# Bardli/RMem_ocu

Measured on AMD Instinct MI355X. Metric: frames/sec (whole node) 480p VOS, N=8 memory bank, higher is better.
Workload: dtype bf16; 1 GPU; davis17_480p_r50_N8; clip_frames=80, job_clips=64, clip_feeder=static, objects=3, memory_bank=1+7, gap=5, clips_in_flight_per_gpu=24, clips_per_group=8, step_unit=batch, parallelism=clip-parallel x1, weights=synthetic (no checkpoint offline), hipgraphs=True, frames_from=HBM, encoder_lookahead=2

## Files before the change

### rmem_ocu_amd/csrc/bottleneck.hip

```cpp
#include "common.h"
#include "lds_dma.h"
#include "../../include/rmem.h"
#include <stdlib.h>

namespace {

constexpr int BM = 64, N1 = 256, BK = 64;
constexpr int R1_BYTES = N1 * BK * 2, CP = 132, R2_BYTES = 16 * CP * 4, R3_BYTES = 32768;
static_assert(R2_BYTES >= BM * BK * 2, "the A panel shares the staging region");
constexpr int LDS_BYTES = R1_BYTES + R2_BYTES + R3_BYTES;

struct BnParams {
  const e16* b; const e16* x2; const e16* w3; const float* b3; const e16* res; e16* y;
  const e16* w1; const float* b1; e16* a2;
  int M, K1, KT, N2;
  int Ho, Wo, HoWo, H2, W2, Cin2, stride2;
  long b_bytes, x2_bytes;
};

template <int N2, bool DUAL>
__global__ __launch_bounds__(256) void k_bneck_chain(BnParams p) {
  constexpr int NB2 = N2 / 32;
  constexpr int NST = N2 == 64 ? 4 : 2;
  constexpr int TN2 = N2 / 32;
  constexpr int NRES = DUAL ? 0 : 8;
  static_assert(NST * N2 * BK * 2 <= R3_BYTES, "W1' ring");
  __shared__ __attribute__((aligned(16))) char smem[LDS_BYTES];
  char* const R1 = smem;
  char* const R2 = smem + R1_BYTES;
  char* const R3 = smem + R1_BYTES + R2_BYTES;

  const int tid = threadIdx.x, lane = tid & 63;
  const int wave = __builtin_amdgcn_readfirstlane(tid >> 6);
  const int wm = wave >> 1, wn = wave & 1;
  const int fr = lane & 15, fc = lane >> 4;
  const int m0 = blockIdx.x * BM;

  int a_off[2], a_off2[2], w3_off[8], w1_off[NB2];
#pragma unroll
  for (int i = 0; i < 2; ++i) {
    const int r = 16 * wave + 8 * i + (lane >> 3);
    const int c = (lane & 7) ^ ((r >> 1) & 7);
    const int m = m0 + r;
    a_off[i] = m < p.M ? (m * p.K1 + c * 8) * 2 : OOB;
    a_off2[i] = OOB;
    if (DUAL && m < p.M) {
      const int img = m / p.HoWo, rem = m - img * p.HoWo;
      const int ho = rem / p.Wo, wo = rem - ho * p.Wo;
      a_off2[i] = (((img * p.H2 + ho * p.stride2) * p.W2 + wo * p.stride2) * p.Cin2 + c * 8) * 2;
    }
  }
#pragma unroll
  for (int i = 0; i < 8; ++i) {
    const int r = 64 * wave + 8 * i + (lane >> 3);
    const int c = (lane & 7) ^ ((r >> 1) & 7);
    w3_off[i] = (r * p.KT + c * 8) * 2;
  }
#pragma unroll
  for (int i = 0; i < NB2; ++i) {
    const int r = (N2 / 4) * wave + 8 * i + (lane >> 3);
    const int c = (lane & 7) ^ ((r >> 1) & 7);
    w1_off[i] = (r * N1 + c * 8) * 2;
  }
  const rsrc_t rs_b = make_rsrc(p.b, p.b_bytes), rs_x2 = make_rsrc(DUAL ? p.x2 : p.b, DUAL ? p.x2_bytes : 0);
  const rsrc_t rs_w3 = make_rsrc(p.w3, (long)N1 * p.KT * 2), rs_w1 = make_rsrc(p.w1, (long)N2 * N1 * 2);
  const int nk1 = p.K1 / BK, nk = p.KT / BK;

  auto issue1 = [&](int kt) {
    if (DUAL && kt >= nk1) {
#pragma unroll
      for (int i = 0; i < 2; ++i) buf_load_lds16(rs_x2, (lptr_t)(R2 + (16 * wave + 8 * i) * 128), a_off2[i], (kt - nk1) * (BK * 2));
    } else {
#pragma unroll
      for (int i = 0; i < 2; ++i) buf_load_lds16(rs_b, (lptr_t)(R2 + (16 * wave + 8 * i) * 128), a_off[i], kt * (BK * 2));
    }
#pragma unroll
    for (int i = 0; i < 8; ++i) buf_load_lds16(rs_w3, (lptr_t)(R1 + (64 * wave + 8 * i) * 128), w3_off[i], kt * (BK * 2));
  };
  auto issue2 = [&](int kt, int stage) {
#pragma unroll
    for (int i = 0; i < NB2; ++i)
      buf_load_lds16(rs_w1, (lptr_t)(R3 + stage * (N2 * BK * 2) + ((N2 / 4) * wave + 8 * i) * 128), w1_off[i], kt * (BK * 2));
  };

  issue1(0);
#pragma unroll
  for (int s = 0; s < NST; ++s) issue2(s, s);
  __builtin_amdgcn_sched_barrier(0);
  e16x8 resv[NRES > 0 ? NRES : 1];
  const int erow = tid >> 4, ecv = tid & 15;
  if constexpr (!DUAL) {
#pragma unroll
    for (int q = 0; q < 8; ++q) {
      const int m = min(m0 + (q >> 1) * 16 + erow, p.M - 1);
      resv[q] = *reinterpret_cast<const e16x8*>(p.res + (long)m * N1 + (q & 1) * 128 + ecv * 8);
    }
  }
  f32x4 bias3[2][2], bias1[2];
#pragma unroll
  for (int h = 0; h < 2; ++h) {
    bias3[h][0] = *reinterpret_cast<const f32x4*>(p.b3 + h * 128 + ecv * 8);
    bias3[h][1] = *reinterpret_cast<const f32x4*>(p.b3 + h * 128 + ecv * 8 + 4);
  }
  constexpr int VPR2 = N2 / 8;
  bias1[0] = *reinterpret_cast<const f32x4*>(p.b1 + (tid % VPR2) * 8);
  bias1[1] = *reinterpret_cast<const f32x4*>(p.b1 + (tid % VPR2) * 8 + 4);
  __builtin_amdgcn_sched_barrier(0);

  f32x4 acc[2][8];
#pragma unroll
  for (int i = 0; i < 2; ++i)
#pragma unroll
    for (int j = 0; j < 8; ++j) acc[i][j] = f32x4{0.f, 0.f, 0.f, 0.f};

  for (int kt = 0; kt < nk; ++kt) {
    if (kt == 0) {
      asm volatile("s_waitcnt vmcnt(%0)" ::"n"(NST * NB2 + NRES + 6) : "memory");
    } else {
      __builtin_amdgcn_s_barrier();
      issue1(kt);
      asm volatile("s_waitcnt vmcnt(0)" ::: "memory");
    }
    __builtin_amdgcn_s_barrier();
    const e16* As = reinterpret_cast<const e16*>(R2);
    const e16* Bs = reinterpret_cast<const e16*>(R1);
#pragma unroll
    for (int ks = 0; ks < 2; ++ks) {
      e16x8 af[2], bfr[8];
#pragma unroll
      for (int i = 0; i < 2; ++i) af[i] = *reinterpret_cast<const e16x8*>(&As[swz(wm * 32 + i * 16 + fr, 4 * ks + fc)]);
#pragma unroll
      for (int j = 0; j < 8; ++j) bfr[j] = *reinterpret_cast<const e16x8*>(&Bs[swz(wn * 128 + j * 16 + fr, 4 * ks + fc)]);
#pragma unroll
      for (int i = 0; i < 2; ++i)
#pragma unroll
        for (int j = 0; j < 8; ++j) acc[i][j] = RMEM_MFMA_16x16x32(af[i], bfr[j], acc[i][j], 0, 0, 0);
    }
  }
  __syncthreads();

  float* Cs = reinterpret_cast<float*>(R2);
  e16* Yt = reinterpret_cast<e16*>(R1);
#pragma unroll
  for (int q = 0; q < 8; ++q) {
    const int g = q >> 1, h = q & 1;
    if (wm == (g >> 1) && wn == h) {
#pragma unroll
      for (int j = 0; j < 8; ++j)
#pragma unroll
        for (int r = 0; r < 4; ++r) Cs[(fc * 4 + r) * CP + j * 16 + fr] = acc[g & 1][j][r];
    }
    __syncthreads();
    {
      const int rt = g * 16 + erow, m = m0 + rt, n = h * 128 + ecv * 8;
      const float* c = Cs + erow * CP + ecv * 8;
      const f32x4 c0 = *reinterpret_cast<const f32x4*>(c), c1 = *reinterpret_cast<const f32x4*>(c + 4);
      const f32x4 b0 = bias3[h][0], b1 = bias3[h][1];
      float v[8] = {c0[0] + b0[0], c0[1] + b0[1], c0[2] + b0[2], c0[3] + b0[3], c1[0] + b1[0], c1[1] + b1[1], c1[2] + b1[2], c1[3] + b1[3]};
      e16x8 o;
#pragma unroll
      for (int j = 0; j < 8; ++j) {
        if constexpr (!DUAL) v[j] += (float)resv[q][j];
        o[j] = (e16)fmaxf(v[j], 0.f);
      }
      if (m < p.M) *reinterpret_cast<e16x8*>(p.y + (long)m * N1 + n) = o;
      *reinterpret_cast<e16x8*>(&Yt[(n >> 6) * (BM * BK) + swz(rt, (n >> 3) & 7)]) = o;
    }
    __syncthreads();
  }

  f32x4 acc2[2][TN2];
#pragma unroll
  for (int i = 0; i < 2; ++i)
#pragma unroll
    for (int j = 0; j < TN2; ++j) acc2[i][j] = f32x4{0.f, 0.f, 0.f, 0.f};
  if constexpr (DUAL) asm volatile("s_waitcnt vmcnt(0)" ::: "memory");
  if constexpr (DUAL) __syncthreads();
#pragma unroll
  for (int kt = 0; kt < 4; ++kt) {
    const int stage = kt % NST;
    if (kt >= NST) {
      if (kt + 1 < 4) asm volatile("s_waitcnt vmcnt(%0)" ::"n"(NB2) : "memory");
      else asm volatile("s_waitcnt vmcnt(0)" ::: "memory");
      __builtin_amdgcn_s_barrier();
    }
    const e16* As = Yt + kt * (BM * BK);
    const e16* Bs = reinterpret_cast<const e16*>(R3 + stage * (N2 * BK * 2));
#pragma unroll
    for (int ks = 0; ks < 2; ++ks) {
      e16x8 af[2], bfr[TN2];
#pragma unroll
      for (int i = 0; i < 2; ++i) af[i] = *reinterpret_cast<const e16x8*>(&As[swz(wm * 32 + i * 16 + fr, 4 * ks + fc)]);
#pragma unroll
      for (int j = 0; j < TN2; ++j) bfr[j] = *reinterpret_cast<const e16x8*>(&Bs[swz(wn * (N2 / 2) + j * 16 + fr, 4 * ks + fc)]);
#pragma unroll
      for (int i = 0; i < 2; ++i)
#pragma unroll
        for (int j = 0; j < TN2; ++j) acc2[i][j] = RMEM_MFMA_16x16x32(af[i], bfr[j], acc2[i][j], 0, 0, 0);
    }
    if (kt + NST < 4) {
      __syncthreads();
      issue2(kt + NST, stage);
    }
  }
  __syncthreads();

  constexpr int CP2 = N2 + 4;
  static_assert(16 * CP2 * 4 <= R2_BYTES, "second staging buffer");
#pragma unroll
  for (int g = 0; g < 4; ++g) {
    if (wm == (g >> 1)) {
#pragma unroll
      for (int j = 0; j < TN2; ++j)
#pragma unroll
        for (int r = 0; r < 4; ++r) Cs[(fc * 4 + r) * CP2 + wn * (N2 / 2) + j * 16 + fr] = acc2[g & 1][j][r];
    }
    __syncthreads();
    if (tid < 16 * VPR2) {
      const int row = tid / VPR2, cv = tid % VPR2;
      const int m = m0 + g * 16 + row, n = cv * 8;
      const float* c = Cs + row * CP2 + n;
      const f32x4 c0 = *reinterpret_cast<const f32x4*>(c), c1 = *reinterpret_cast<const f32x4*>(c + 4);
      const f32x4 b0 = bias1[0], b1 = bias1[1];
      const float v[8] = {c0[0] + b0[0], c0[1] + b0[1], c0[2] + b0[2], c0[3] + b0[3], c1[0] + b1[0], c1[1] + b1[1], c1[2] + b1[2], c1[3] + b1[3]};
      e16x8 o;
#pragma unroll
      for (int j = 0; j < 8; ++j) o[j] = (e16)fmaxf(v[j], 0.f);
      if (m < p.M) *reinterpret_cast<e16x8*>(p.a2 + (long)m * N2 + n) = o;
    }
    __syncthreads();
  }
}

bool al16(const void* q) { return ((uintptr_t)q % 16) == 0; }

}

extern "C" int RMEM_API(rmem_bneck_chain)(const rmem_bneck_chain_desc* d, const void* b, const void* x2, const void* w3, const float* bias3,
                                          const void* res, void* y, const void* w1, const float* bias1, void* a2, void* stream) {
  RMEM_REQUIRE(d && b && w3 && bias3 && y && w1 && bias1 && a2, "rmem_bneck_chain: null argument");
  RMEM_REQUIRE(d->batch >= 1 && d->Ho > 0 && d->Wo > 0 && d->K1 > 0 && d->K1 % 64 == 0 && d->Cout == 256 && (d->N2 == 64 || d->N2 == 128),
               "rmem_bneck_chain: K1 must be a multiple of 64, Cout 256, N2 64 or 128");
  RMEM_REQUIRE((x2 != nullptr) != (res != nullptr), "rmem_bneck_chain: exactly one of res (identity shortcut) and x2 (1x1 shortcut) must be given");
  RMEM_REQUIRE(!x2 || (d->Cin2 > 0 && d->Cin2 % 64 == 0 && d->stride2 >= 1 && d->H2 >= (d->Ho - 1) * d->stride2 + 1 && d->W2 >= (d->Wo - 1) * d->stride2 + 1),
               "rmem_bneck_chain: the 1x1 shortcut needs Cin2 % 64 == 0 and an H2 x W2 map that covers the strided samples");
  RMEM_REQUIRE(al16(b) && al16(x2) && al16(w3) && al16(bias3) && al16(res) && al16(y) && al16(w1) && al16(bias1) && al16(a2),
               "rmem_bneck_chain: operands must be 16-byte aligned");
  BnParams p;
  p.b = (const e16*)b; p.x2 = (const e16*)x2; p.w3 = (const e16*)w3; p.b3 = bias3; p.res = (const e16*)res; p.y = (e16*)y;
  p.w1 = (const e16*)w1; p.b1 = bias1; p.a2 = (e16*)a2;
  p.Ho = d->Ho; p.Wo = d->Wo; p.HoWo = d->Ho * d->Wo;
  const long M = (long)d->batch * p.HoWo;
  p.K1 = d->K1; p.KT = d->K1 + (x2 ? d->Cin2 : 0); p.N2 = d->N2;
  p.H2 = d->H2; p.W2 = d->W2; p.Cin2 = d->Cin2; p.stride2 = d->stride2;
  p.b_bytes = M * d->K1 * 2;
  p.x2_bytes = x2 ? (long)d->batch * d->H2 * d->W2 * d->Cin2 * 2 : 0;
  const long lim = (1L << 31) - (1L << 22);
  RMEM_REQUIRE(M < (1L << 30) && p.b_bytes < lim && p.x2_bytes < lim, "rmem_bneck_chain: an operand exceeds the 2 GB a buffer descriptor addresses");
  p.M = (int)M;
  const dim3 grid((unsigned)((M + BM - 1) / BM));
  hipStream_t s = (hipStream_t)stream;
  if (x2) {
    if (d->N2 == 64) hipLaunchKernelGGL((k_bneck_chain<64, true>), grid, dim3(256), 0, s, p);
    else hipLaunchKernelGGL((k_bneck_chain<128, true>), grid, dim3(256), 0, s, p);
  } else {
    if (d->N2 == 64) hipLaunchKernelGGL((k_bneck_chain<64, false>), grid, dim3(256), 0, s, p);
    else hipLaunchKernelGGL((k_bneck_chain<128, false>), grid, dim3(256), 0, s, p);
  }
  return rmem_check_launch("rmem_bneck_chain");
}
```

### rmem_ocu_amd/encoder_batch.py

```python
from __future__ import annotations

import os
from typing import Dict, Tuple

import torch

from . import ops
from .pack import R50_BLOCKS, R50_STRIDES
from .runtime import BF16, F32, _out


class _PtrInput:

    def _init_ptrs(self, B: int, device):
        self.img_ptrs = torch.tensor([self.img_in[i].data_ptr() for i in range(B)], dtype=torch.int64).to(device)
        self._ptr_ring = ops.PinnedRing(4, (B,), torch.int64, device)
        self._ptrs_set = False

    def _input_op(self):
        return ops.image_ptrs_to_nhwc8(self.img_ptrs, self.img8, H=self.H, W=self.W, images=self.B)

    def set_frames(self, frames, stream: int):
        assert len(frames) == self.B
        host = self._ptr_ring.next()
        for i, f in enumerate(frames):
            assert f.dtype == F32 and f.is_contiguous() and f.numel() == 3 * self.H * self.W
            host[i] = f.data_ptr()
        self._ptr_ring.upload(self.img_ptrs, self.B * 8, stream)
        self._ptrs_set = True

    def point_at_img_in(self, stream: int):
        if self._ptrs_set:
            self.set_frames([self.img_in[i] for i in range(self.B)], stream)
            self._ptrs_set = False


class BatchEncoder(_PtrInput):
    def __init__(self, P: Dict[str, torch.Tensor], in_hw: Tuple[int, int], batch: int, device):
        if 'pe.w' in P:
            raise ops.RmemError('BatchEncoder covers the ResNet-50 encoder')
        self.P, self.B, self.dev = P, batch, device
        H, W = in_hw
        self.H, self.W = H, W
        B = batch
        self.H2, self.W2 = _out(H, 7, 2, 3), _out(W, 7, 2, 3)
        self.H4, self.W4 = _out(self.H2, 3, 2, 1), _out(self.W2, 3, 2, 1)
        self.H8, self.W8 = _out(self.H4, 3, 2, 1), _out(self.W4, 3, 2, 1)
        self.H16, self.W16 = _out(self.H8, 3, 2, 1), _out(self.W8, 3, 2, 1)
        M4, M8, L = self.H4 * self.W4, self.H8 * self.W8, self.H16 * self.W16
        dt16 = P['stem.w'].dtype
        e = lambda *shape, dt=None: torch.empty(*shape, dtype=dt or dt16, device=device)
        self.img_in = e(B, 3, H, W, dt=F32)
        self._init_ptrs(B, device)
        self.stem4 = os.environ.get('RMEM_STEM', 'pool') != 'rowrun' and 'stem.w4' in P
        if self.stem4:
            hp, wp = ops.stem_padded_size(H, W)
            self.img4 = torch.zeros(B, hp, wp, 4, dtype=dt16, device=device)
        else:
            self.img8 = e(B, H * W, 8)
        self.stem_pool = self.stem4 and os.environ.get('RMEM_STEM', 'pool') == 'pool'
        self.stem = None if self.stem_pool else e(B, self.H2 * self.W2, 64)
        self.pool = e(B, M4, 64)
        self.x4 = [e(B, M4, 256), e(B, M4, 256)]
        self.x8 = [e(B, M8, 512), e(B, M8, 512)]
        self.x16 = [e(B, L, 1024), e(B, L, 1024)]
        self.mid_a = e(B * M4 * 128)
        self.mid_b = e(B * M4 * 64)
        self.conv_ws = torch.empty(16 * B * L * 256, dtype=F32, device=device)
        self._prog = None
        self.enc_out = (self.x4[(R50_BLOCKS[0] - 1) % 2], self.x8[(R50_BLOCKS[1] - 1) % 2], self.x16[(R50_BLOCKS[2] - 1) % 2])

    def _conv(self, *a, **kw):
        return ops.conv2d(*a, ws=self.conv_ws, batch=self.B, **kw)

    def prog(self) -> list:
        if self._prog is not None:
            return self._prog
        P, B, o = self.P, self.B, []
        nsplit = int(os.environ.get('RMEM_ENC_FRONT_SPLIT', '1'))
        if nsplit < 1 or B % nsplit:
            nsplit = 1
        chain_on = os.environ.get('RMEM_NO_BNECK_CHAIN', '0') != '1'
        block_on = chain_on and os.environ.get('RMEM_NO_BNECK_BLOCK', '0') != '1'
        direct3 = () if os.environ.get('RMEM_NO_DIRECT_CONV3', '0') == '1' else ((64, 128) if os.environ.get('RMEM_DIRECT_CONV3_128') == '1' else (64,))
        blocks = [(li, bi) for li, nblk in enumerate(R50_BLOCKS, start=1) for bi in range(nblk)]
        outs = [self.x4, self.x8, self.x16]
        M4 = self.H4 * self.W4
        if nsplit > 1 and getattr(self, 'mid_a128', None) is None:
            self.mid_a128 = torch.empty(B * M4 * 128, dtype=self.pool.dtype, device=self.dev)

        def sub(t, per_image, b0, nb):
            return t.reshape(-1)[b0 * per_image:(b0 + nb) * per_image]

        def stem(b0, nb):
            q = []
            conv = lambda *a_, **kw: ops.conv2d(*a_, ws=self.conv_ws, batch=nb, **kw)
            pool = sub(self.pool, M4 * 64, b0, nb)
            if self.stem4:
                hp, wp = ops.stem_padded_size(self.H, self.W)
                img4 = sub(self.img4, hp * wp * 4, b0, nb)
                q.append(ops.image_ptrs_to_nhwc4p(self.img_ptrs[b0:], img4, H=self.H, W=self.W, images=nb))
                if self.stem_pool:
                    q.append(ops.stem7x7s2_pool(img4, P['stem.w4'], P['stem.b'], pool, H=self.H, W=self.W, images=nb))
                else:
                    st = sub(self.stem, self.H2 * self.W2 * 64, b0, nb)
                    q.append(ops.stem7x7s2(img4, P['stem.w4'], P['stem.b'], st, H=self.H, W=self.W, images=nb))
                    q.append(ops.maxpool3x3s2(st, pool, H=self.H2, W=self.W2, C=64, images=nb))
            else:
                img8 = sub(self.img8, self.H * self.W * 8, b0, nb)
                st = sub(self.stem, self.H2 * self.W2 * 64, b0, nb)
                q.append(ops.image_ptrs_to_nhwc8(self.img_ptrs[b0:], img8, H=self.H, W=self.W, images=nb))
                q.append(conv(img8, P['stem.w'], P['stem.b'], st, H=self.H, W=self.W, Cin=8, Cout=64, KH=7, KW=7, stride=2, pad=3, relu=True))
                q.append(ops.maxpool3x3s2(st, pool, H=self.H2, W=self.W2, C=64, images=nb))
            return q

        def run_blocks(idxs, b0, nb, x, hw, cin, conv1_done):
            q = []
            conv = lambda *a_, **kw: ops.conv2d(*a_, ws=self.conv_ws, batch=nb, **kw)
            h, w = hw
            for idx in idxs:
                li, bi = blocks[idx]
                stride = R50_STRIDES[li - 1]
                planes = 64 * 2 ** (li - 1)
                p = f'encoder.layer{li}.{bi}'
                s = stride if bi == 0 else 1
                ho, wo = _out(h, 3, s, 1), _out(w, 3, s, 1)
                xs = sub(x, h * w * cin, b0, nb)
                y = sub(outs[li - 1][bi % 2], ho * wo * planes * 4, b0, nb)
                abuf = self.mid_a128 if (nsplit > 1 and li == 2 and bi == 0) else self.mid_a
                a = sub(abuf, h * w * planes, b0, nb)
                bb = sub(self.mid_b, ho * wo * planes, b0, nb)
                dual = (p + '.c3ds.w') in P
                nxt = blocks[idx + 1] if idx + 1 < len(blocks) else None
                if block_on and li == 1 and s == 1 and not conv1_done and cin == (64 if dual else 256):
                    kw = {}
                    if nxt == (2, 0):
                        pn = 'encoder.layer2.0'
                        nbuf = self.mid_a128 if nsplit > 1 else self.mid_a
                        kw = dict(w1n=P[pn + '.conv1.w'], bias1n=P[pn + '.conv1.b'], a_next=sub(nbuf, ho * wo * 128, b0, nb))
                        conv1_done = True
                    q.append(ops.bneck_block64(xs, P[p + '.conv1.w'], P[p + '.conv1.b'], P[p + '.conv2.w'], P[p + '.conv2.b'],
                                               P[p + ('.c3ds.w' if dual else '.conv3.w')], P[p + ('.c3ds.b' if dual else '.conv3.b')], y,
                                               H=h, W=w, Cin=cin, images=nb, **kw))
                    x, (h, w), cin = outs[li - 1][bi % 2], (ho, wo), planes * 4
                    continue
                if not conv1_done:
                    q.append(conv(xs, P[p + '.conv1.w'], P[p + '.conv1.b'], a, H=h, W=w, Cin=cin, Cout=planes, relu=True))
                conv1_done = False
                if planes in direct3 and s == 1:
                    q.append(ops.conv3x3_direct(a, P[p + '.conv2.w'], P[p + '.conv2.b'], bb, H=h, W=w, C=planes, images=nb, relu=True))
                else:
                    q.append(conv(a, P[p + '.conv2.w'], P[p + '.conv2.b'], bb, H=h, W=w, Cin=planes, Cout=planes, KH=3, KW=3, stride=s, pad=1,
                                  relu=True))
                if chain_on and li == 1 and nxt is not None:
                    pn = f'encoder.layer{nxt[0]}.{nxt[1]}'
                    n2 = 64 * 2 ** (nxt[0] - 1)
                    nbuf = self.mid_a128 if (nsplit > 1 and nxt == (2, 0)) else self.mid_a
                    a_next = sub(nbuf, ho * wo * n2, b0, nb)
                    kw = dict(x2=xs, H2=h, W2=w, Cin2=cin, stride2=s) if dual else dict(residual=xs)
                    q.append(ops.bneck_chain(bb, P[p + ('.c3ds.w' if dual else '.conv3.w')], P[p + ('.c3ds.b' if dual else '.conv3.b')], y,
                                             P[pn + '.conv1.w'], P[pn + '.conv1.b'], a_next, H=ho, W=wo, K1=planes, N2=n2, batch=nb, **kw))
                    conv1_done = True
                elif dual:
                    q.append(ops.conv1x1_dual(bb, xs, P[p + '.c3ds.w'], P[p + '.c3ds.b'], y, H=ho, W=wo, Cin=planes, Cout=planes * 4,
                                              H2=h, W2=w, Cin2=cin, stride2=s, relu=True, batch=nb))
                else:
                    q.append(conv(bb, P[p + '.conv3.w'], P[p + '.conv3.b'], y, H=ho, W=wo, Cin=planes, Cout=planes * 4, residual=xs, relu=True))
                x, (h, w), cin = outs[li - 1][bi % 2], (ho, wo), planes * 4
            return q, x, (h, w), cin, conv1_done

        n1 = R50_BLOCKS[0]
        nb = B // nsplit
        for k in range(nsplit):
            o += stem(k * nb, nb)
            q, x, hw, cin, c1 = run_blocks(range(n1), k * nb, nb, self.pool, (self.H4, self.W4), 64, False)
            o += q
        q, x, hw, cin, c1 = run_blocks(range(n1, len(blocks)), 0, B, x, hw, cin, c1)
        o += q
        self._prog = o
        return o


class SwinBatchEncoder(_PtrInput):

    def __init__(self, P: Dict[str, torch.Tensor], in_hw: Tuple[int, int], batch: int, device):
        if 'pe.w' not in P:
            raise ops.RmemError('SwinBatchEncoder covers the Swin-B encoder')
        self.P, self.B, self.dev = P, batch, device
        H, W = in_hw
        if H % 4 or W % 4:
            raise ops.RmemError('Swin-B path: network size must be a multiple of 4')
        self.H, self.W = H, W
        B = batch
        self.H4, self.W4 = H // 4, W // 4
        self.H8, self.W8 = (self.H4 + 1) // 2, (self.W4 + 1) // 2
        self.H16, self.W16 = (self.H8 + 1) // 2, (self.W8 + 1) // 2
        M4, M8, L = self.H4 * self.W4, self.H8 * self.W8, self.H16 * self.W16
        dt16 = P['proj.w'].dtype
        e = lambda *shape, dt=None: torch.empty(*shape, dtype=dt or dt16, device=device)
        self.img_in = e(B, 3, H, W, dt=F32)
        self._init_ptrs(B, device)
        self.img8 = e(B, H * W, 8)
        self.sx = e(B * M4, 128, dt=F32)
        self.sln = e(B * M4, 128)
        self.sqkv = e(B * M4, 384)
        self.satt = e(B * M4, 128)
        self.smlp = e(B * M4, 512)
        self.smerge = e(B * M8, 512)
        self.enc_out = (e(B, M4, 128), e(B, M8, 256), e(B, L, 512))
        self.conv_ws = torch.empty(16 * B * L * 256, dtype=F32, device=device)
        self._prog = None

    def _lin(self, x, name, y, M, K, N, **kw):
        return ops.linear(x, self.P[name + '.w'], self.P[name + '.b'], y, M=M, K=K, N=N, ws=self.conv_ws, **kw)

    def prog(self) -> list:
        if self._prog is not None:
            return self._prog
        from .pack import SWIN_DEPTHS, SWIN_HEADS
        P, B, o = self.P, self.B, []
        o.append(self._input_op())
        h, w, C = self.H4, self.W4, 128
        x = self.sx.view(-1)
        o.append(ops.conv2d(self.img8, P['pe.w'], P['pe.b'], x[: B * h * w * C], H=self.H, W=self.W, Cin=8, Cout=C, KH=4, KW=4, stride=4,
                            batch=B))
        o.append(ops.layernorm(x, P['pe.ln.g'], P['pe.ln.b'], M=B * h * w, C=C, yf=x))
        for li, (depth, heads) in enumerate(zip(SWIN_DEPTHS, SWIN_HEADS)):
            M = h * w
            ln, qkv, att, mlp = self.sln.view(-1), self.sqkv.view(-1), self.satt.view(-1), self.smlp.view(-1)
            for b in range(depth):
                d = f'sw{li}.{b}'
                o.append(ops.layernorm(x, P[d + '.norm1.g'], P[d + '.norm1.b'], M=B * M, C=C, y=ln))
                o.append(self._lin(ln, d + '.qkv', qkv, B * M, C, 3 * C))
                o.append(ops.window_attn(qkv, P[d + '.qkv.b'], P[d + '.table'], att, H=h, W=w, C=C, heads=heads,
                                         shift=0 if b % 2 == 0 else 3, images=B))
                o.append(self._lin(att, d + '.proj', x, B * M, C, C, residual=x))
                o.append(ops.layernorm(x, P[d + '.norm2.g'], P[d + '.norm2.b'], M=B * M, C=C, y=ln))
                o.append(self._lin(ln, d + '.fc1', mlp, B * M, C, 4 * C, relu=2))
                o.append(self._lin(mlp, d + '.fc2', x, B * M, 4 * C, C, residual=x))
            o.append(ops.layernorm(x, P[f'sw.norm{li}.g'], P[f'sw.norm{li}.b'], M=B * M, C=C, y=self.enc_out[li]))
            if li < len(SWIN_DEPTHS) - 1:
                mg = self.smerge.view(-1)
                h2, w2 = (h + 1) // 2, (w + 1) // 2
                o.append(ops.patch_merge_ln(x, P[f'sw{li}.merge.g'], P[f'sw{li}.merge.b'], mg, H=h, W=w, C=C, images=B))
# ... 6 lines not shown
```

### rmem_ocu_amd/ops.py

```python
from __future__ import annotations

import ctypes as C
import os
from typing import Dict, Optional, Sequence

import torch

from . import _lib
from ._lib import AttnChunk, ConvDesc, RmemError

BF16 = torch.bfloat16
F16 = torch.float16
F32 = torch.float32
E16 = (BF16, F16)


def _fn(name: str, dt):
    if dt not in E16:
        raise RmemError(f'{name}: 16-bit operands must be bfloat16 or float16, got {dt}')
    return getattr(_lib.lib(), name + ('_f16' if dt == F16 else ''))


def _first16(*ts):
    for t in ts:
# ... 2 lines not shown
    return BF16


class Op:
    __slots__ = ('fn', 'args', 'name', 'keep')

    def __init__(self, fn, args, name, keep=()):
        self.fn, self.args, self.name, self.keep = fn, args, name, keep

    def __call__(self, stream: int):
        rc = self.fn(*self.args, stream)
        if rc:
            raise RmemError(f'{self.name} failed ({rc}): {_lib.lib().rmem_last_error_string().decode()}')


def run(ops, stream: Optional[int] = None):
    if stream is None:
        stream = torch.cuda.current_stream().cuda_stream
    if isinstance(ops, Op):
        ops(stream)
    else:
        for o in ops:
            o(stream)


def _ptr(t: Optional[torch.Tensor]):
    return None if t is None else t.data_ptr()


def _dev(*ts):
    for t in ts:
        if t is not None and not t.is_cuda:
            raise RmemError('librmem_hip ops need device tensors (no CPU fallback)')


def conv2d(x, w, bias, y, *, H, W, Cin, Cout, KH=1, KW=1, stride=1, pad=0, residual=None, y2=None, relu=False,
           ldo=None, ldr=None, ld2=None, ws=None, ldx=0, act_begin=0, batch=1, res_up=None) -> Op:
    _dev(x, w, bias, y, residual, y2)
    dt = w.dtype
    assert x.dtype == dt and w.dtype == dt and w.is_contiguous()
    assert w.numel() == Cout * KH * KW * Cin, (w.shape, Cout, KH, KW, Cin)
    assert bias is None or (bias.dtype == F32 and bias.numel() == Cout)
    assert y.dtype in (dt, F32) and (y2 is None or y2.dtype == dt)
    Ho = (H + 2 * pad - KH) // stride + 1
    Wo = (W + 2 * pad - KW) // stride + 1
    ldo = Cout if ldo is None else ldo
    ldr = Cout if ldr is None else ldr
    ld2 = Cout if ld2 is None else ld2
    assert x.numel() >= (batch * H * W - 1) * (ldx or Cin) + Cin and y.numel() >= (batch * Ho * Wo - 1) * ldo + Cout
    assert batch == 1 or not ldx
    ru = (0, 0, 0) if res_up is None else (int(res_up[0]), int(res_up[1]), int(bool(res_up[2])))
    if res_up is not None:
        assert residual is not None and residual.dtype == dt and residual.numel() >= (batch * ru[0] * ru[1] - 1) * ldr + Cout
    d = ConvDesc(H, W, Cin, Ho, Wo, Cout, KH, KW, stride, pad, ldo, ldr, ld2, int(relu), int(y.dtype == F32),
                 int(residual is not None and residual.dtype == F32), ldx, batch, act_begin, *ru)
    if ws is not None:
        _dev(ws)
        if ws.numel() * ws.element_size() < _lib.lib().rmem_conv_workspace_bytes(C.byref(d)):
            ws = None
    args = (C.byref(d), _ptr(x), _ptr(w), _ptr(bias), _ptr(residual), _ptr(y), _ptr(y2), _ptr(ws))
    return Op(_fn('rmem_conv2d_nhwc', dt), args, 'rmem_conv2d_nhwc', (d, x, w, bias, residual, y, y2, ws))


def conv_plan(*, H, W, Cin, Cout, KH=1, KW=1, stride=1, pad=0, batch=1, ldx=0, has_ws=False, entry='conv2d', extra=0) -> Dict[str, int]:
    Ho = (H + 2 * pad - KH) // stride + 1
    Wo = (W + 2 * pad - KW) // stride + 1
    d = ConvDesc(H, W, Cin, Ho, Wo, Cout, KH, KW, stride, pad, Cout, Cout, Cout, 0, 0, 0, ldx, batch, 0, 0, 0, 0)
    pl = _lib.GemmPlan()
    _lib.check(_lib.lib().rmem_conv_plan(C.byref(d), int(has_ws), _lib.GEMM_ENTRIES.index(entry), extra, C.byref(pl)), 'rmem_conv_plan')
    return {n: getattr(pl, n) for n, _ in pl._fields_}


def conv1x1_dual(x, x2, w_cat, bias, y, *, H, W, Cin, Cout, H2, W2, Cin2, stride2, relu=False, batch=1) -> Op:
    _dev(x, x2, w_cat, bias, y)
    dt = w_cat.dtype
    assert x.dtype == dt and x2.dtype == dt and w_cat.dtype == dt and w_cat.is_contiguous() and y.dtype == dt
    assert w_cat.numel() == Cout * (Cin + Cin2) and bias.dtype == F32 and bias.numel() == Cout
    assert x.numel() >= batch * H * W * Cin and x2.numel() >= batch * H2 * W2 * Cin2 and y.numel() >= batch * H * W * Cout
    d = ConvDesc(H, W, Cin, H, W, Cout, 1, 1, 1, 0, Cout, Cout, Cout, int(relu), 0, 0, 0, batch, 0, 0, 0, 0)
    args = (C.byref(d), _ptr(x), _ptr(x2), H2, W2, Cin2, stride2, _ptr(w_cat), _ptr(bias), _ptr(y))
    return Op(_fn('rmem_conv1x1_dual_nhwc', dt), args, 'rmem_conv1x1_dual_nhwc', (d, x, x2, w_cat, bias, y))


def bneck_chain(b, w3, bias3, y, w1, bias1, a2, *, H, W, K1, N2, residual=None, x2=None, H2=0, W2=0, Cin2=0, stride2=1, batch=1) -> Op:
    _dev(b, w3, bias3, y, w1, bias1, a2, residual, x2)
    dt = w3.dtype
    M = batch * H * W
    assert (residual is None) != (x2 is None)
    assert all(t.dtype == dt for t in (b, y, w1, a2)) and bias3.dtype == F32 and bias1.dtype == F32
    assert w3.is_contiguous() and w1.is_contiguous() and w3.numel() == 256 * (K1 + (Cin2 if x2 is not None else 0)) and w1.numel() == N2 * 256
    assert b.numel() >= M * K1 and y.numel() >= M * 256 and a2.numel() >= M * N2 and bias3.numel() == 256 and bias1.numel() == N2
    assert residual is None or (residual.dtype == dt and residual.numel() >= M * 256)
    assert x2 is None or (x2.dtype == dt and x2.numel() >= batch * H2 * W2 * Cin2)
    d = _lib.BneckChainDesc(batch, H, W, K1, 256, N2, H2, W2, Cin2, stride2)
    args = (C.byref(d), _ptr(b), _ptr(x2), _ptr(w3), _ptr(bias3), _ptr(residual), _ptr(y), _ptr(w1), _ptr(bias1), _ptr(a2))
    return Op(_fn('rmem_bneck_chain', dt), args, 'rmem_bneck_chain', (d, b, x2, w3, bias3, residual, y, w1, bias1, a2))


def bneck_block64(x, w1, bias1, w2, bias2, w3, bias3, y, *, H, W, Cin, images, w1n=None, bias1n=None, a_next=None) -> Op:
    _dev(x, w1, bias1, w2, bias2, w3, bias3, y, w1n, bias1n, a_next)
    dt = w1.dtype
    M = images * H * W
    tail = w1n is not None
    assert Cin in (64, 256) and (not tail or Cin == 256) and (bias1n is not None) == tail and (a_next is not None) == tail
    assert all(t.dtype == dt for t in (x, w2, w3, y)) and all(t.dtype == F32 for t in (bias1, bias2, bias3))
    assert w1.is_contiguous() and w2.is_contiguous() and w3.is_contiguous()
    assert w1.numel() == 64 * Cin and w2.numel() == 64 * 9 * 64 and w3.numel() == 256 * (64 if Cin == 256 else 128)
    assert bias1.numel() == 64 and bias2.numel() == 64 and bias3.numel() == 256
    assert x.numel() >= M * Cin and y.numel() >= M * 256
    if tail:
        assert w1n.dtype == dt and a_next.dtype == dt and bias1n.dtype == F32 and w1n.is_contiguous()
        assert w1n.numel() == 128 * 256 and bias1n.numel() == 128 and a_next.numel() >= M * 128
    d = _lib.BneckBlockDesc(images, H, W, Cin, 128 if tail else 0)
    args = (C.byref(d), _ptr(x), _ptr(w1), _ptr(bias1), _ptr(w2), _ptr(bias2), _ptr(w3), _ptr(bias3), _ptr(y), _ptr(w1n), _ptr(bias1n), _ptr(a_next))
    return Op(_fn('rmem_bneck_block64', dt), args, 'rmem_bneck_block64', (d, x, w1, bias1, w2, bias2, w3, bias3, y, w1n, bias1n, a_next))


def linear(x, w, bias, y, *, M, K, N, residual=None, y2=None, relu=False, ldo=None, ldr=None, ld2=None, ws=None, ldx=0,
           act_begin=0) -> Op:
    return conv2d(x, w, bias, y, H=M, W=1, Cin=K, Cout=N, residual=residual, y2=y2, relu=relu, ldo=ldo, ldr=ldr, ld2=ld2, ws=ws,
                  ldx=ldx, act_begin=act_begin)


def _ptr_array(ts):
    return (C.c_void_p * len(ts))(*[_ptr(t) for t in ts])


def linear_grouped(xs, ws, biases, ys, *, M, K, N, residuals=None, relu=False) -> Op:
    n = len(xs)
    assert 1 <= n <= 4 and len(ws) == n and len(ys) == n and (biases is None or len(biases) == n)
    _dev(*xs, *ws, *ys, *(biases or ()), *(residuals or ()))
    dt = ws[0].dtype
    for x, w, y in zip(xs, ws, ys):
        assert x.dtype == dt and w.dtype == dt and w.numel() == N * K and x.numel() >= M * K and y.numel() >= M * N
    assert len({y.dtype for y in ys}) == 1 and (residuals is None or len({r.dtype for r in residuals}) == 1)
    d = ConvDesc(M, 1, K, M, 1, N, 1, 1, 1, 0, N, N, N, int(relu), int(ys[0].dtype == F32),
                 int(residuals is not None and residuals[0].dtype == F32), 0, 1, 0)
    arrs = (_ptr_array(xs), _ptr_array(ws), _ptr_array(biases) if biases is not None else None,
            _ptr_array(residuals) if residuals is not None else None, _ptr_array(ys))
    args = (C.byref(d), n, arrs[0], arrs[1], arrs[2], arrs[3], arrs[4])
    return Op(_fn('rmem_linear_grouped', dt), args, 'rmem_linear_grouped', (d, arrs, xs, ws, biases, residuals, ys))


def add16_grouped(as_, bs, ys, n: int) -> Op:
    _dev(*as_, *bs, *ys)
    dt = as_[0].dtype
    assert len(as_) == len(bs) == len(ys) <= 8 and all(t.dtype == dt for t in (*as_, *bs, *ys))
    arrs = (_ptr_array(as_), _ptr_array(bs), _ptr_array(ys))
    return Op(_fn('rmem_add16_grouped', dt), (len(as_), arrs[0], arrs[1], arrs[2], n), 'rmem_add16_grouped', (arrs, as_, bs, ys))


def layernorm256_pair(a0, b0, y0, a1, b1, y1, gamma, beta, *, M, eps=1e-5) -> Op:
    _dev(a0, b0, y0, a1, b1, y1, gamma, beta)
    dt = a0.dtype
    assert all(t.dtype == dt and t.numel() >= M * 256 for t in (a0, b0, y0, a1, b1, y1)) and gamma.dtype == F32
    args = (_ptr(a0), _ptr(b0), _ptr(y0), _ptr(a1), _ptr(b1), _ptr(y1), _ptr(gamma), _ptr(beta), eps, M)
    return Op(_fn('rmem_layernorm256_pair', dt), args, 'rmem_layernorm256_pair', (a0, b0, y0, a1, b1, y1, gamma, beta))


def lstt_chain_rows(L: int, clips: int, cus: int) -> int:
    return int(_lib.lib().rmem_lstt_chain_rows(int(L), int(clips), int(cus)))


def attn_merge():
    return _lib.AttnMerge()


def _chain(name, cls, ints, ptrs, dt, extra=()):
    ts = list(ptrs.values())
    _dev(*ts)
    for k, t in ptrs.items():
        if t is not None and t.data_ptr() % 16:
            raise RmemError(f'{name}: {k} must be 16-byte aligned')
    d = cls(int(ints[0]), int(ints[1]), float(ints[2]), int(ints[3]), *[_ptr(t) for t in ts])
    return Op(_fn(name, dt), (C.byref(d), *[C.byref(e) for e in extra]), name, (d, ts, extra))


# ... 541 lines not shown
```

Measured before the change: 3423 frames/s.

## Extend fused bottleneck conv3+next-conv1 chain kernel to layer2 (Cout 512)

Generalizes the fused bottleneck chain kernel, which computes the conv3 output (plus residual or 1x1 shortcut) and immediately feeds it into the next block's conv1. It now handles Cout=512 by processing two 256-channel chunks per tile and accumulating the conv1 GEMM across both. Layer-2 blocks now use this path instead of a separate conv3 kernel followed by a conv1 kernel, which avoids re-reading the 512-channel activation and saves a launch. In exchange the kernel carries more register pressure (launch_bounds with 2 waves per SIMD, a split B-fragment loop) and a more complex wait/barrier schedule.

```diff
diff --git a/rmem_ocu_amd/csrc/bottleneck.hip b/rmem_ocu_amd/csrc/bottleneck.hip
--- a/rmem_ocu_amd/csrc/bottleneck.hip
+++ b/rmem_ocu_amd/csrc/bottleneck.hip
@@ -18,12 +18,16 @@
   long b_bytes, x2_bytes;
 };
 
-template <int N2, bool DUAL>
-__global__ __launch_bounds__(256) void k_bneck_chain(BnParams p) {
+template <int N2, bool DUAL, int NCH>
+__global__ __launch_bounds__(256, NCH) void k_bneck_chain(BnParams p) {
+  constexpr int COUT = N1 * NCH;
   constexpr int NB2 = N2 / 32;
-  constexpr int NST = N2 == 64 ? 4 : 2;
+  constexpr int NST = R3_BYTES / (N2 * BK * 2) < 4 * NCH ? R3_BYTES / (N2 * BK * 2) : 4 * NCH;
+  constexpr int NK2 = 4 * NCH;
   constexpr int TN2 = N2 / 32;
   constexpr int NRES = DUAL ? 0 : 8;
+  constexpr int JB = N2 == 256 ? (DUAL ? 4 : 2) : 8;
+  static_assert(NST >= 1 && NST <= 4, "W1' ring");
   static_assert(NST * N2 * BK * 2 <= R3_BYTES, "W1' ring");
   __shared__ __attribute__((aligned(16))) char smem[LDS_BYTES];
   char* const R1 = smem;
@@ -36,7 +40,7 @@
   const int fr = lane & 15, fc = lane >> 4;
   const int m0 = blockIdx.x * BM;
 
-  int a_off[2], a_off2[2], w3_off[8], w1_off[NB2];
+  int a_off[2], a_off2[2], w3_off[2], w1_off[2];
 #pragma unroll
   for (int i = 0; i < 2; ++i) {
     const int r = 16 * wave + 8 * i + (lane >> 3);
@@ -51,22 +55,22 @@
     }
   }
 #pragma unroll
-  for (int i = 0; i < 8; ++i) {
+  for (int i = 0; i < 2; ++i) {
     const int r = 64 * wave + 8 * i + (lane >> 3);
     const int c = (lane & 7) ^ ((r >> 1) & 7);
     w3_off[i] = (r * p.KT + c * 8) * 2;
   }
 #pragma unroll
-  for (int i = 0; i < NB2; ++i) {
+  for (int i = 0; i < 2; ++i) {
     const int r = (N2 / 4) * wave + 8 * i + (lane >> 3);
     const int c = (lane & 7) ^ ((r >> 1) & 7);
-    w1_off[i] = (r * N1 + c * 8) * 2;
+    w1_off[i] = (r * COUT + c * 8) * 2;
   }
   const rsrc_t rs_b = make_rsrc(p.b, p.b_bytes), rs_x2 = make_rsrc(DUAL ? p.x2 : p.b, DUAL ? p.x2_bytes : 0);
-  const rsrc_t rs_w3 = make_rsrc(p.w3, (long)N1 * p.KT * 2), rs_w1 = make_rsrc(p.w1, (long)N2 * N1 * 2);
+  const rsrc_t rs_w3 = make_rsrc(p.w3, (long)COUT * p.KT * 2), rs_w1 = make_rsrc(p.w1, (long)N2 * COUT * 2);
   const int nk1 = p.K1 / BK, nk = p.KT / BK;
 
-  auto issue1 = [&](int kt) {
+  auto issue1 = [&](int kt, int ch) {
     if (DUAL && kt >= nk1) {
 #pragma unroll
       for (int i = 0; i < 2; ++i) buf_load_lds16(rs_x2, (lptr_t)(R2 + (16 * wave + 8 * i) * 128), a_off2[i], (kt - nk1) * (BK * 2));
@@ -75,150 +79,183 @@
       for (int i = 0; i < 2; ++i) buf_load_lds16(rs_b, (lptr_t)(R2 + (16 * wave + 8 * i) * 128), a_off[i], kt * (BK * 2));
     }
 #pragma unroll
-    for (int i = 0; i < 8; ++i) buf_load_lds16(rs_w3, (lptr_t)(R1 + (64 * wave + 8 * i) * 128), w3_off[i], kt * (BK * 2));
+    for (int i = 0; i < 8; ++i)
+      buf_load_lds16(rs_w3, (lptr_t)(R1 + (64 * wave + 8 * i) * 128), w3_off[i & 1], (ch * N1 + (i >> 1) * 16) * 2 * p.KT + kt * (BK * 2));
   };
   auto issue2 = [&](int kt, int stage) {
 #pragma unroll
     for (int i = 0; i < NB2; ++i)
-      buf_load_lds16(rs_w1, (lptr_t)(R3 + stage * (N2 * BK * 2) + ((N2 / 4) * wave + 8 * i) * 128), w1_off[i], kt * (BK * 2));
-  };
-
-  issue1(0);
+      buf_load_lds16(rs_w1, (lptr_t)(R3 + stage * (N2 * BK * 2) + ((N2 / 4) * wave + 8 * i) * 128), w1_off[i & 1], (i >> 1) * 16 * COUT * 2 + kt * (BK * 2));
+  };
+
+  issue1(0, 0);
 #pragma unroll
   for (int s = 0; s < NST; ++s) issue2(s, s);
   __builtin_amdgcn_sched_barrier(0);
   e16x8 resv[NRES > 0 ? NRES : 1];
+  f32x4 bias3[2][2], bias1[2];
   const int erow = tid >> 4, ecv = tid & 15;
-  if constexpr (!DUAL) {
-#pragma unroll
-    for (int q = 0; q < 8; ++q) {
-      const int m = min(m0 + (q >> 1) * 16 + erow, p.M - 1);
-      resv[q] = *reinterpret_cast<const e16x8*>(p.res + (long)m * N1 + (q & 1) * 128 + ecv * 8);
-    }
-  }
-  f32x4 bias3[2][2], bias1[2];
-#pragma unroll
-  for (int h = 0; h < 2; ++h) {
-    bias3[h][0] = *reinterpret_cast<const f32x4*>(p.b3 + h * 128 + ecv * 8);
-    bias3[h][1] = *reinterpret_cast<const f32x4*>(p.b3 + h * 128 + ecv * 8 + 4);
-  }
+  auto load_res = [&](int ch) {
+    if constexpr (!DUAL) {
+#pragma unroll
+      for (int q = 0; q < 8; ++q) {
+        const int m = min(m0 + (q >> 1) * 16 + erow, p.M - 1);
+        resv[q] = *reinterpret_cast<const e16x8*>(p.res + (long)m * COUT + ch * N1 + (q & 1) * 128 + ecv * 8);
+      }
+    }
+  };
+  auto load_bias3 = [&](int ch) {
+#pragma unroll
+    for (int h = 0; h < 2; ++h) {
+      bias3[h][0] = *reinterpret_cast<const f32x4*>(p.b3 + ch * N1 + h * 128 + ecv * 8);
+      bias3[h][1] = *reinterpret_cast<const f32x4*>(p.b3 + ch * N1 + h * 128 + ecv * 8 + 4);
+    }
+  };
+  load_res(0);
+  load_bias3(0);
   constexpr int VPR2 = N2 / 8;
-  bias1[0] = *reinterpret_cast<const f32x4*>(p.b1 + (tid % VPR2) * 8);
-  bias1[1] = *reinterpret_cast<const f32x4*>(p.b1 + (tid % VPR2) * 8 + 4);
+  auto load_bias1 = [&]() {
+    bias1[0] = *reinterpret_cast<const f32x4*>(p.b1 + (tid % VPR2) * 8);
+    bias1[1] = *reinterpret_cast<const f32x4*>(p.b1 + (tid % VPR2) * 8 + 4);
+  };
+  constexpr int NB1 = NCH == 1 ? 2 : 0;
+  if constexpr (NB1 != 0) load_bias1();
   __builtin_amdgcn_sched_barrier(0);
 
-  f32x4 acc[2][8];
+  f32x4 acc2[2][TN2];
 #pragma unroll
   for (int i = 0; i < 2; ++i)
 #pragma unroll
-    for (int j = 0; j < 8; ++j) acc[i][j] = f32x4{0.f, 0.f, 0.f, 0.f};
-
-  for (int kt = 0; kt < nk; ++kt) {
-    if (kt == 0) {
-      asm volatile("s_waitcnt vmcnt(%0)" ::"n"(NST * NB2 + NRES + 6) : "memory");
-    } else {
-      __builtin_amdgcn_s_barrier();
-      issue1(kt);
-      asm volatile("s_waitcnt vmcnt(0)" ::: "memory");
-    }
-    __builtin_amdgcn_s_barrier();
-    const e16* As = reinterpret_cast<const e16*>(R2);
-    const e16* Bs = reinterpret_cast<const e16*>(R1);
-#pragma unroll
-    for (int ks = 0; ks < 2; ++ks) {
-      e16x8 af[2], bfr[8];
-#pragma unroll
-      for (int i = 0; i < 2; ++i) af[i] = *reinterpret_cast<const e16x8*>(&As[swz(wm * 32 + i * 16 + fr, 4 * ks + fc)]);
-#pragma unroll
-      for (int j = 0; j < 8; ++j) bfr[j] = *reinterpret_cast<const e16x8*>(&Bs[swz(wn * 128 + j * 16 + fr, 4 * ks + fc)]);
-#pragma unroll
-      for (int i = 0; i < 2; ++i)
-#pragma unroll
-        for (int j = 0; j < 8; ++j) acc[i][j] = RMEM_MFMA_16x16x32(af[i], bfr[j], acc[i][j], 0, 0, 0);
-    }
-  }
-  __syncthreads();
-
+    for (int j = 0; j < TN2; ++j) acc2[i][j] = f32x4{0.f, 0.f, 0.f, 0.f};
   float* Cs = reinterpret_cast<float*>(R2);
   e16* Yt = reinterpret_cast<e16*>(R1);
-#pragma unroll
-  for (int q = 0; q < 8; ++q) {
-    const int g = q >> 1, h = q & 1;
-    if (wm == (g >> 1) && wn == h) {
-#pragma unroll
-      for (int j = 0; j < 8; ++j)
-#pragma unroll
-        for (int r = 0; r < 4; ++r) Cs[(fc * 4 + r) * CP + j * 16 + fr] = acc[g & 1][j][r];
+
+#pragma unroll
+  for (int ch = 0; ch < NCH; ++ch) {
+    f32x4 acc[2][8];
+#pragma unroll
+    for (int i = 0; i < 2; ++i)
+#pragma unroll
+      for (int j = 0; j < 8; ++j) acc[i][j] = f32x4{0.f, 0.f, 0.f, 0.f};
+
+    for (int kt = 0; kt < nk; ++kt) {
+      if (ch == 0 && kt == 0) {
+        asm volatile("s_waitcnt vmcnt(%0)" ::"n"(NST * NB2 + NRES + 4 + NB1) : "memory");
+      } else {
+        __builtin_amdgcn_s_barrier();
+        issue1(kt, ch);
+        if (ch > 0 && kt == 0) {
+          load_res(ch);
+          load_bias3(ch);
+        }
+        asm volatile("s_waitcnt vmcnt(0)" ::: "memory");
+      }
+      __builtin_amdgcn_s_barrier();
+      const e16* As = reinterpret_cast<const e16*>(R2);
+      const e16* Bs = reinterpret_cast<const e16*>(R1);
+#pragma unroll
+      for (int ks = 0; ks < 2; ++ks) {
+        e16x8 af[2], bfr[JB];
+#pragma unroll
+        for (int i = 0; i < 2; ++i) af[i] = *reinterpret_cast<const e16x8*>(&As[swz(wm * 32 + i * 16 + fr, 4 * ks + fc)]);
+#pragma unroll
+        for (int j0 = 0; j0 < 8; j0 += JB) {
+#pragma unroll
+          for (int j = 0; j < JB; ++j) bfr[j] = *reinterpret_cast<const e16x8*>(&Bs[swz(wn * 128 + (j0 + j) * 16 + fr, 4 * ks + fc)]);
+#pragma unroll
+          for (int i = 0; i < 2; ++i)
+#pragma unroll
+            for (int j = 0; j < JB; ++j) acc[i][j0 + j] = RMEM_MFMA_16x16x32(af[i], bfr[j], acc[i][j0 + j], 0, 0, 0);
+        }
+      }
     }
     __syncthreads();
-    {
-      const int rt = g * 16 + erow, m = m0 + rt, n = h * 128 + ecv * 8;
-      const float* c = Cs + erow * CP + ecv * 8;
-      const f32x4 c0 = *reinterpret_cast<const f32x4*>(c), c1 = *reinterpret_cast<const f32x4*>(c + 4);
-      const f32x4 b0 = bias3[h][0], b1 = bias3[h][1];
-      float v[8] = {c0[0] + b0[0], c0[1] + b0[1], c0[2] + b0[2], c0[3] + b0[3], c1[0] + b1[0], c1[1] + b1[1], c1[2] + b1[2], c1[3] + b1[3]};
-      e16x8 o;
-#pragma unroll
-      for (int j = 0; j < 8; ++j) {
-        if constexpr (!DUAL) v[j] += (float)resv[q][j];
-        o[j] = (e16)fmaxf(v[j], 0.f);
-      }
-      if (m < p.M) *reinterpret_cast<e16x8*>(p.y + (long)m * N1 + n) = o;
-      *reinterpret_cast<e16x8*>(&Yt[(n >> 6) * (BM * BK) + swz(rt, (n >> 3) & 7)]) = o;
+
+#pragma unroll
+    for (int q = 0; q < 8; ++q) {
+      const int g = q >> 1, h = q & 1;
+      if (wm == (g >> 1) && wn == h) {
+#pragma unroll
+        for (int j = 0; j < 8; ++j)
+#pragma unroll
+          for (int r = 0; r < 4; ++r) Cs[(fc * 4 + r) * CP + j * 16 + fr] = acc[g & 1][j][r];
+      }
+      __syncthreads();
+      {
+        const int rt = g * 16 + erow, m = m0 + rt, n = h * 128 + ecv * 8;
+        const float* c = Cs + erow * CP + ecv * 8;
+        const f32x4 c0 = *reinterpret_cast<const f32x4*>(c), c1 = *reinterpret_cast<const f32x4*>(c + 4);
+        const f32x4 b0 = bias3[h][0], b1 = bias3[h][1];
+        float v[8] = {c0[0] + b0[0], c0[1] + b0[1], c0[2] + b0[2], c0[3] + b0[3], c1[0] + b1[0], c1[1] + b1[1], c1[2] + b1[2], c1[3] + b1[3]};
+        e16x8 o;
+#pragma unroll
+        for (int j = 0; j < 8; ++j) {
+          if constexpr (!DUAL) v[j] += (float)resv[q][j];
+          o[j] = (e16)fmaxf(v[j], 0.f);
+        }
+        if (m < p.M) *reinterpret_cast<e16x8*>(p.y + (long)m * COUT + ch * N1 + n) = o;
+        *reinterpret_cast<e16x8*>(&Yt[(n >> 6) * (BM * BK) + swz(rt, (n >> 3) & 7)]) = o;
+      }
+      __syncthreads();
+    }
+
+    if constexpr (DUAL) {
+      if (ch == 0) {
+        asm volatile("s_waitcnt vmcnt(0)" ::: "memory");
+        __syncthreads();
+      }
+    }
+    if (NB1 == 0 && ch == NCH - 1) load_bias1();
+#pragma unroll
+    for (int kt = 0; kt < 4; ++kt) {
+      const int g = ch * 4 + kt, stage = g % NST;
+      if (kt >= NST) {
+        if (NST == 2 && g + 1 < NK2) asm volatile("s_waitcnt vmcnt(%0)" ::"n"(NB2) : "memory");
+        else asm volatile("s_waitcnt vmcnt(0)" ::: "memory");
+        __builtin_amdgcn_s_barrier();
+      }
+      const e16* As = Yt + kt * (BM * BK);
+      const e16* Bs = reinterpret_cast<const e16*>(R3 + stage * (N2 * BK * 2));
+#pragma unroll
+      for (int ks = 0; ks < 2; ++ks) {
+        constexpr int JB2 = TN2 < JB ? TN2 : JB;
+        e16x8 af[2], bfr[JB2];
+#pragma unroll
+        for (int i = 0; i < 2; ++i) af[i] = *reinterpret_cast<const e16x8*>(&As[swz(wm * 32 + i * 16 + fr, 4 * ks + fc)]);
+#pragma unroll
+        for (int j0 = 0; j0 < TN2; j0 += JB2) {
+#pragma unroll
+          for (int j = 0; j < JB2; ++j) bfr[j] = *reinterpret_cast<const e16x8*>(&Bs[swz(wn * (N2 / 2) + (j0 + j) * 16 + fr, 4 * ks + fc)]);
+#pragma unroll
+          for (int i = 0; i < 2; ++i)
+#pragma unroll
+            for (int j = 0; j < JB2; ++j) acc2[i][j0 + j] = RMEM_MFMA_16x16x32(af[i], bfr[j], acc2[i][j0 + j], 0, 0, 0);
+        }
+      }
+      if (g + NST < NK2) {
+        __syncthreads();
+        issue2(g + NST, stage);
+      }
+    }
+  }
+  __syncthreads();
+
+  constexpr int CP2 = N2 + 4;
+  constexpr int RP2 = N2 == 256 ? 8 : 16;
+  static_assert(RP2 * CP2 * 4 <= R2_BYTES && RP2 * VPR2 <= 256, "second staging buffer");
+#pragma unroll
+  for (int gp = 0; gp < BM / RP2; ++gp) {
+    const int g = gp * RP2 / 16, hr = gp % (16 / RP2);
+    if (wm == (g >> 1) && (RP2 == 16 || (fc >> 1) == hr)) {
+#pragma unroll
+      for (int j = 0; j < TN2; ++j)
+#pragma unroll
+        for (int r = 0; r < 4; ++r) Cs[(fc * 4 % RP2 + r) * CP2 + wn * (N2 / 2) + j * 16 + fr] = acc2[g & 1][j][r];
     }
     __syncthreads();
-  }
-
-  f32x4 acc2[2][TN2];
-#pragma unroll
-  for (int i = 0; i < 2; ++i)
-#pragma unroll
-    for (int j = 0; j < TN2; ++j) acc2[i][j] = f32x4{0.f, 0.f, 0.f, 0.f};
-  if constexpr (DUAL) asm volatile("s_waitcnt vmcnt(0)" ::: "memory");
-  if constexpr (DUAL) __syncthreads();
-#pragma unroll
-  for (int kt = 0; kt < 4; ++kt) {
-    const int stage = kt % NST;
-    if (kt >= NST) {
-      if (kt + 1 < 4) asm volatile("s_waitcnt vmcnt(%0)" ::"n"(NB2) : "memory");
-      else asm volatile("s_waitcnt vmcnt(0)" ::: "memory");
-      __builtin_amdgcn_s_barrier();
-    }
-    const e16* As = Yt + kt * (BM * BK);
-    const e16* Bs = reinterpret_cast<const e16*>(R3 + stage * (N2 * BK * 2));
-#pragma unroll
-    for (int ks = 0; ks < 2; ++ks) {
-      e16x8 af[2], bfr[TN2];
-#pragma unroll
-      for (int i = 0; i < 2; ++i) af[i] = *reinterpret_cast<const e16x8*>(&As[swz(wm * 32 + i * 16 + fr, 4 * ks + fc)]);
-#pragma unroll
-      for (int j = 0; j < TN2; ++j) bfr[j] = *reinterpret_cast<const e16x8*>(&Bs[swz(wn * (N2 / 2) + j * 16 + fr, 4 * ks + fc)]);
-#pragma unroll
-      for (int i = 0; i < 2; ++i)
-#pragma unroll
-        for (int j = 0; j < TN2; ++j) acc2[i][j] = RMEM_MFMA_16x16x32(af[i], bfr[j], acc2[i][j], 0, 0, 0);
-    }
-    if (kt + NST < 4) {
-      __syncthreads();
-      issue2(kt + NST, stage);
-    }
-  }
-  __syncthreads();
-
-  constexpr int CP2 = N2 + 4;
-  static_assert(16 * CP2 * 4 <= R2_BYTES, "second staging buffer");
-#pragma unroll
-  for (int g = 0; g < 4; ++g) {
-    if (wm == (g >> 1)) {
-#pragma unroll
-      for (int j = 0; j < TN2; ++j)
-#pragma unroll
-        for (int r = 0; r < 4; ++r) Cs[(fc * 4 + r) * CP2 + wn * (N2 / 2) + j * 16 + fr] = acc2[g & 1][j][r];
-    }
-    __syncthreads();
-    if (tid < 16 * VPR2) {
+    if (tid < RP2 * VPR2) {
       const int row = tid / VPR2, cv = tid % VPR2;
-      const int m = m0 + g * 16 + row, n = cv * 8;
+      const int m = m0 + gp * RP2 + row, n = cv * 8;
       const float* c = Cs + row * CP2 + n;
       const f32x4 c0 = *reinterpret_cast<const f32x4*>(c), c1 = *reinterpret_cast<const f32x4*>(c + 4);
       const f32x4 b0 = bias1[0], b1 = bias1[1];
@@ -239,8 +276,9 @@
 extern "C" int RMEM_API(rmem_bneck_chain)(const rmem_bneck_chain_desc* d, const void* b, const void* x2, const void* w3, const float* bias3,
                                           const void* res, void* y, const void* w1, const float* bias1, void* a2, void* stream) {
   RMEM_REQUIRE(d && b && w3 && bias3 && y && w1 && bias1 && a2, "rmem_bneck_chain: null argument");
-  RMEM_REQUIRE(d->batch >= 1 && d->Ho > 0 && d->Wo > 0 && d->K1 > 0 && d->K1 % 64 == 0 && d->Cout == 256 && (d->N2 == 64 || d->N2 == 128),
-               "rmem_bneck_chain: K1 must be a multiple of 64, Cout 256, N2 64 or 128");
+  RMEM_REQUIRE(d->batch >= 1 && d->Ho > 0 && d->Wo > 0 && d->K1 > 0 && d->K1 % 64 == 0 &&
+               ((d->Cout == 256 && (d->N2 == 64 || d->N2 == 128)) || (d->Cout == 512 && (d->N2 == 128 || d->N2 == 256))),
+               "rmem_bneck_chain: K1 must be a multiple of 64; Cout 256 with N2 64 or 128, or Cout 512 with N2 128 or 256");
   RMEM_REQUIRE((x2 != nullptr) != (res != nullptr), "rmem_bneck_chain: exactly one of res (identity shortcut) and x2 (1x1 shortcut) must be given");
   RMEM_REQUIRE(!x2 || (d->Cin2 > 0 && d->Cin2 % 64 == 0 && d->stride2 >= 1 && d->H2 >= (d->Ho - 1) * d->stride2 + 1 && d->W2 >= (d->Wo - 1) * d->stride2 + 1),
                "rmem_bneck_chain: the 1x1 shortcut needs Cin2 % 64 == 0 and an H2 x W2 map that covers the strided samples");
@@ -256,16 +294,24 @@
   p.b_bytes = M * d->K1 * 2;
   p.x2_bytes = x2 ? (long)d->batch * d->H2 * d->W2 * d->Cin2 * 2 : 0;
   const long lim = (1L << 31) - (1L << 22);
-  RMEM_REQUIRE(M < (1L << 30) && p.b_bytes < lim && p.x2_bytes < lim, "rmem_bneck_chain: an operand exceeds the 2 GB a buffer descriptor addresses");
+  RMEM_REQUIRE(M * d->Cout < (1L << 31) && p.b_bytes < lim && p.x2_bytes < lim, "rmem_bneck_chain: an operand exceeds the 2 GB a buffer descriptor addresses");
   p.M = (int)M;
   const dim3 grid((unsigned)((M + BM - 1) / BM));
   hipStream_t s = (hipStream_t)stream;
-  if (x2) {
-    if (d->N2 == 64) hipLaunchKernelGGL((k_bneck_chain<64, true>), grid, dim3(256), 0, s, p);
-    else hipLaunchKernelGGL((k_bneck_chain<128, true>), grid, dim3(256), 0, s, p);
+  if (d->Cout == 512) {
+    if (x2) {
+      if (d->N2 == 128) hipLaunchKernelGGL((k_bneck_chain<128, true, 2>), grid, dim3(256), 0, s, p);
+      else hipLaunchKernelGGL((k_bneck_chain<256, true, 2>), grid, dim3(256), 0, s, p);
+    } else {
+      if (d->N2 == 128) hipLaunchKernelGGL((k_bneck_chain<128, false, 2>), grid, dim3(256), 0, s, p);
+      else hipLaunchKernelGGL((k_bneck_chain<256, false, 2>), grid, dim3(256), 0, s, p);
+    }
+  } else if (x2) {
+    if (d->N2 == 64) hipLaunchKernelGGL((k_bneck_chain<64, true, 1>), grid, dim3(256), 0, s, p);
+    else hipLaunchKernelGGL((k_bneck_chain<128, true, 1>), grid, dim3(256), 0, s, p);
   } else {
-    if (d->N2 == 64) hipLaunchKernelGGL((k_bneck_chain<64, false>), grid, dim3(256), 0, s, p);
-    else hipLaunchKernelGGL((k_bneck_chain<128, false>), grid, dim3(256), 0, s, p);
+    if (d->N2 == 64) hipLaunchKernelGGL((k_bneck_chain<64, false, 1>), grid, dim3(256), 0, s, p);
+    else hipLaunchKernelGGL((k_bneck_chain<128, false, 1>), grid, dim3(256), 0, s, p);
   }
   return rmem_check_launch("rmem_bneck_chain");
 }
diff --git a/rmem_ocu_amd/encoder_batch.py b/rmem_ocu_amd/encoder_batch.py
--- a/rmem_ocu_amd/encoder_batch.py
+++ b/rmem_ocu_amd/encoder_batch.py
@@ -82,6 +82,7 @@
             nsplit = 1
         chain_on = os.environ.get('RMEM_NO_BNECK_CHAIN', '0') != '1'
         block_on = chain_on and os.environ.get('RMEM_NO_BNECK_BLOCK', '0') != '1'
+        chain2_on = chain_on and os.environ.get('RMEM_NO_BNECK_CHAIN2', '0') != '1'
         direct3 = () if os.environ.get('RMEM_NO_DIRECT_CONV3', '0') == '1' else ((64, 128) if os.environ.get('RMEM_DIRECT_CONV3_128') == '1' else (64,))
         blocks = [(li, bi) for li, nblk in enumerate(R50_BLOCKS, start=1) for bi in range(nblk)]
         outs = [self.x4, self.x8, self.x16]
@@ -152,14 +153,14 @@
                 else:
                     q.append(conv(a, P[p + '.conv2.w'], P[p + '.conv2.b'], bb, H=h, W=w, Cin=planes, Cout=planes, KH=3, KW=3, stride=s, pad=1,
                                   relu=True))
-                if chain_on and li == 1 and nxt is not None:
+                if ((chain_on and li == 1) or (chain2_on and li == 2)) and nxt is not None:
                     pn = f'encoder.layer{nxt[0]}.{nxt[1]}'
                     n2 = 64 * 2 ** (nxt[0] - 1)
                     nbuf = self.mid_a128 if (nsplit > 1 and nxt == (2, 0)) else self.mid_a
                     a_next = sub(nbuf, ho * wo * n2, b0, nb)
                     kw = dict(x2=xs, H2=h, W2=w, Cin2=cin, stride2=s) if dual else dict(residual=xs)
                     q.append(ops.bneck_chain(bb, P[p + ('.c3ds.w' if dual else '.conv3.w')], P[p + ('.c3ds.b' if dual else '.conv3.b')], y,
-                                             P[pn + '.conv1.w'], P[pn + '.conv1.b'], a_next, H=ho, W=wo, K1=planes, N2=n2, batch=nb, **kw))
+                                             P[pn + '.conv1.w'], P[pn + '.conv1.b'], a_next, H=ho, W=wo, K1=planes, N2=n2, batch=nb, Cout=planes * 4, **kw))
                     conv1_done = True
                 elif dual:
                     q.append(ops.conv1x1_dual(bb, xs, P[p + '.c3ds.w'], P[p + '.c3ds.b'], y, H=ho, W=wo, Cin=planes, Cout=planes * 4,
diff --git a/rmem_ocu_amd/ops.py b/rmem_ocu_amd/ops.py
--- a/rmem_ocu_amd/ops.py
+++ b/rmem_ocu_amd/ops.py
@@ -108,17 +108,19 @@
     return Op(_fn('rmem_conv1x1_dual_nhwc', dt), args, 'rmem_conv1x1_dual_nhwc', (d, x, x2, w_cat, bias, y))
 
 
-def bneck_chain(b, w3, bias3, y, w1, bias1, a2, *, H, W, K1, N2, residual=None, x2=None, H2=0, W2=0, Cin2=0, stride2=1, batch=1) -> Op:
+def bneck_chain(b, w3, bias3, y, w1, bias1, a2, *, H, W, K1, N2, residual=None, x2=None, H2=0, W2=0, Cin2=0, stride2=1, batch=1,
+                Cout=256) -> Op:
     _dev(b, w3, bias3, y, w1, bias1, a2, residual, x2)
     dt = w3.dtype
     M = batch * H * W
     assert (residual is None) != (x2 is None)
     assert all(t.dtype == dt for t in (b, y, w1, a2)) and bias3.dtype == F32 and bias1.dtype == F32
-    assert w3.is_contiguous() and w1.is_contiguous() and w3.numel() == 256 * (K1 + (Cin2 if x2 is not None else 0)) and w1.numel() == N2 * 256
-    assert b.numel() >= M * K1 and y.numel() >= M * 256 and a2.numel() >= M * N2 and bias3.numel() == 256 and bias1.numel() == N2
-    assert residual is None or (residual.dtype == dt and residual.numel() >= M * 256)
+    assert (Cout, N2) in ((256, 64), (256, 128), (512, 128), (512, 256))
+    assert w3.is_contiguous() and w1.is_contiguous() and w3.numel() == Cout * (K1 + (Cin2 if x2 is not None else 0)) and w1.numel() == N2 * Cout
+    assert b.numel() >= M * K1 and y.numel() >= M * Cout and a2.numel() >= M * N2 and bias3.numel() == Cout and bias1.numel() == N2
+    assert residual is None or (residual.dtype == dt and residual.numel() >= M * Cout)
     assert x2 is None or (x2.dtype == dt and x2.numel() >= batch * H2 * W2 * Cin2)
-    d = _lib.BneckChainDesc(batch, H, W, K1, 256, N2, H2, W2, Cin2, stride2)
+    d = _lib.BneckChainDesc(batch, H, W, K1, Cout, N2, H2, W2, Cin2, stride2)
     args = (C.byref(d), _ptr(b), _ptr(x2), _ptr(w3), _ptr(bias3), _ptr(residual), _ptr(y), _ptr(w1), _ptr(bias1), _ptr(a2))
     return Op(_fn('rmem_bneck_chain', dt), args, 'rmem_bneck_chain', (d, b, x2, w3, bias3, residual, y, w1, bias1, a2))
 
```

Measured after the change: 3474 frames/s (median of 6 runs). +1.5%, better.
